# NVlabs/GLAMR

Hardware: NVIDIA H100
Metric: global_opt_frame_person_iterations_per_sec (higher is better)
Workload: dtype f32

## Files before the change

### glamr_b200/csrc/common.cuh

```cuda
#pragma once
#include <cuda_fp16.h>
#include <cuda_runtime.h>
#include <stdint.h>
#include <stdio.h>
#include <stdlib.h>

#include "../../include/glamr_b200.h"

#define GLAMR_CUDA_TRY(expr)                       \
  do {                                             \
    cudaError_t _e = (expr);                       \
    if (_e != cudaSuccess) return (int)_e;         \
  } while (0)

#define GLAMR_LAUNCH_CHECK()                       \
  do {                                             \
    cudaError_t _e = cudaGetLastError();           \
    if (_e != cudaSuccess) return (int)_e;         \
  } while (0)

#ifdef GLAMR_EXPERIMENT
#define GLAMR_DBG(x) (x)
#else
#define GLAMR_DBG(x) 0
// ... 42 lines not shown
}
__device__ __forceinline__ void mbar_fence_init() { asm volatile("fence.mbarrier_init.release.cluster;" ::: "memory"); }
__device__ __forceinline__ void mbar_expect_tx(uint64_t* bar, uint32_t bytes) {
  asm volatile("mbarrier.arrive.expect_tx.shared::cta.b64 _, [%0], %1;" ::"r"(smem_u32(bar)), "r"(bytes) : "memory");
}
__device__ __forceinline__ void mbar_expect_tx_only(uint64_t* bar, uint32_t bytes) {
  asm volatile("mbarrier.expect_tx.relaxed.cta.shared::cta.b64 [%0], %1;" ::"r"(smem_u32(bar)), "r"(bytes) : "memory");
}
__device__ __forceinline__ void mbar_arrive(uint64_t* bar) {
  asm volatile("mbarrier.arrive.shared::cta.b64 _, [%0];" ::"r"(smem_u32(bar)) : "memory");
}
__device__ __forceinline__ void mbar_wait(uint64_t* bar, uint32_t parity) {
  uint32_t ok = 0;
  const uint32_t addr = smem_u32(bar);
  while (!ok) {
    asm volatile(
        "{\n\t.reg .pred p;\n\t"
        "mbarrier.try_wait.parity.shared::cta.b64 p, [%1], %2;\n\t"
        "selp.u32 %0, 1, 0, p;\n\t}"
        : "=r"(ok)
        : "r"(addr), "r"(parity)
        : "memory");
  }
}
__device__ __forceinline__ void tma_bulk_g2s(void* smem_dst, const void* gsrc, uint32_t bytes, uint64_t* bar) {
  asm volatile("cp.async.bulk.shared::cluster.global.mbarrier::complete_tx::bytes [%0], [%1], %2, [%3];" ::"r"(smem_u32(smem_dst)),
               "l"(gsrc), "r"(bytes), "r"(smem_u32(bar))
               : "memory");
}

__device__ __forceinline__ void pdl_wait() { asm volatile("griddepcontrol.wait;" ::: "memory"); }
__device__ __forceinline__ void pdl_launch_dependents() { asm volatile("griddepcontrol.launch_dependents;" ::: "memory"); }

__device__ __forceinline__ uint64_t wgmma_desc_kmajor_noswizzle(const void* smem_ptr, int rows) {
  const uint32_t addr = smem_u32(smem_ptr);
  uint64_t d = 0;
  d |= (uint64_t)((addr >> 4) & 0x3FFF);
  d |= (uint64_t)((rows * 16) >> 4) << 16;
  d |= (uint64_t)(128 >> 4) << 32;
  return d;
}
__device__ __forceinline__ void wgmma_fence() { asm volatile("wgmma.fence.sync.aligned;" ::: "memory"); }
__device__ __forceinline__ void wgmma_commit() { asm volatile("wgmma.commit_group.sync.aligned;" ::: "memory"); }
template <int N>
__device__ __forceinline__ void wgmma_wait() { asm volatile("wgmma.wait_group.sync.aligned %0;" ::"n"(N) : "memory"); }
template <int R>
__device__ __forceinline__ void wgmma_fence_acc(float (&d)[R]) {
#pragma unroll
  for (int i = 0; i < R; ++i) asm volatile("" : "+f"(d[i])::"memory");
}
__device__ __forceinline__ void wgmma_m64n128k8_tf32(float (&d)[64], uint64_t da, uint64_t db, uint32_t accumulate) {
  asm volatile(
      "{\n\t.reg .pred p;\n\tsetp.ne.b32 p, %66, 0;\n\t"
      "wgmma.mma_async.sync.aligned.m64n128k8.f32.tf32.tf32 "
      "{%0, %1, %2, %3, %4, %5, %6, %7, %8, %9, %10, %11, %12, %13, %14, %15, %16, %17, %18, %19, %20, %21, %22, %23, %24, %25, %26, %27, %28, %29, %30, %31, %32, %33, %34, %35, %36, %37, %38, %39, %40, %41, %42, %43, %44, %45, %46, %47, %48, %49, %50, %51, %52, %53, %54, %55, %56, %57, %58, %59, %60, %61, %62, %63}, %64, %65, p, 1, 1;\n\t}\n"
      : "+f"(d[0]), "+f"(d[1]), "+f"(d[2]), "+f"(d[3]), "+f"(d[4]), "+f"(d[5]), "+f"(d[6]), "+f"(d[7]),
        "+f"(d[8]), "+f"(d[9]), "+f"(d[10]), "+f"(d[11]), "+f"(d[12]), "+f"(d[13]), "+f"(d[14]), "+f"(d[15]),
        "+f"(d[16]), "+f"(d[17]), "+f"(d[18]), "+f"(d[19]), "+f"(d[20]), "+f"(d[21]), "+f"(d[22]), "+f"(d[23]),
        "+f"(d[24]), "+f"(d[25]), "+f"(d[26]), "+f"(d[27]), "+f"(d[28]), "+f"(d[29]), "+f"(d[30]), "+f"(d[31]),
        "+f"(d[32]), "+f"(d[33]), "+f"(d[34]), "+f"(d[35]), "+f"(d[36]), "+f"(d[37]), "+f"(d[38]), "+f"(d[39]),
        "+f"(d[40]), "+f"(d[41]), "+f"(d[42]), "+f"(d[43]), "+f"(d[44]), "+f"(d[45]), "+f"(d[46]), "+f"(d[47]),
        "+f"(d[48]), "+f"(d[49]), "+f"(d[50]), "+f"(d[51]), "+f"(d[52]), "+f"(d[53]), "+f"(d[54]), "+f"(d[55]),
        "+f"(d[56]), "+f"(d[57]), "+f"(d[58]), "+f"(d[59]), "+f"(d[60]), "+f"(d[61]), "+f"(d[62]), "+f"(d[63])
      : "l"(da), "l"(db), "r"(accumulate));
}
__device__ __forceinline__ void wgmma_m64n240k8_tf32(float (&d)[120], uint64_t da, uint64_t db, uint32_t accumulate) {
// ... 53 lines not shown
        "+f"(d[96]), "+f"(d[97]), "+f"(d[98]), "+f"(d[99]), "+f"(d[100]), "+f"(d[101]), "+f"(d[102]), "+f"(d[103]),
        "+f"(d[104]), "+f"(d[105]), "+f"(d[106]), "+f"(d[107]), "+f"(d[108]), "+f"(d[109]), "+f"(d[110]), "+f"(d[111]),
        "+f"(d[112]), "+f"(d[113]), "+f"(d[114]), "+f"(d[115]), "+f"(d[116]), "+f"(d[117]), "+f"(d[118]), "+f"(d[119]),
        "+f"(d[120]), "+f"(d[121]), "+f"(d[122]), "+f"(d[123]), "+f"(d[124]), "+f"(d[125]), "+f"(d[126]), "+f"(d[127])
      : "l"(da), "l"(db), "r"(accumulate));
}


__device__ __forceinline__ void split_tf32(float x, float& hi, float& lo) {
  uint32_t h, l;
  asm("cvt.rna.tf32.f32 %0, %1;" : "=r"(h) : "f"(x));
  hi = __uint_as_float(h);
  asm("cvt.rna.tf32.f32 %0, %1;" : "=r"(l) : "f"(x - hi));
  lo = __uint_as_float(l);
}
__device__ __forceinline__ void split_f16_scaled(float x, float s, __half& hi, __half& lo) {
  const float xs = x * s;
  hi = __float2half_rn(xs);
  lo = __float2half_rn(xs - __half2float(hi));
}

__device__ __forceinline__ float warp_sum(float v) {
#pragma unroll
  for (int o = 16; o > 0; o >>= 1) v += __shfl_xor_sync(0xffffffffu, v, o);
  return v;
}
__device__ __forceinline__ double warp_sum(double v) {
#pragma unroll
  for (int o = 16; o > 0; o >>= 1) v += __shfl_xor_sync(0xffffffffu, v, o);
  return v;
}

#if defined(__CUDACC__)
constexpr int kPdlDefaultMask = 0;
inline bool pdl_enabled(int bit) {
  static int mask = -1;
  if (mask < 0) {
    const char* e = getenv("GLAMR_PDL");
    mask = e ? atoi(e) : kPdlDefaultMask;
  }
  return (mask & bit) != 0;
}
template <typename... KArgs, typename... Args>
inline cudaError_t launch_pdl(int bit, void (*kernel)(KArgs...), dim3 grid, dim3 block, size_t smem, cudaStream_t s, Args... args) {
  cudaLaunchConfig_t cfg = {};
  cfg.gridDim = grid;
  cfg.blockDim = block;
  cfg.dynamicSmemBytes = smem;
  cfg.stream = s;
  cudaLaunchAttribute attr[1];
  attr[0].id = cudaLaunchAttributeProgrammaticStreamSerialization;
  attr[0].val.programmaticStreamSerializationAllowed = 1;
  cfg.attrs = attr;
  cfg.numAttrs = pdl_enabled(bit) ? 1 : 0;
  return cudaLaunchKernelEx(&cfg, kernel, KArgs(args)...);
}
#endif

}
```

### glamr_b200/csrc/globalopt_kernels.cu

```cuda
#include <stdlib.h>
#include <algorithm>
#include <string.h>
#include <vector>

#include "globalopt_frames.cuh"
#include "smpl_model.cuh"
#include "block_scan.cuh"

namespace glamr {

constexpr int kFrameThreads = 128;

struct GroupGrid {
  int res0;
  int cam0;
  int cam30;
  int slot0;
};
struct SlotLayout {
  int res;
  int persons;
  int cam;
  int cam3;
  int n_res, n_cam, n_cam3;
// ... 21 lines not shown
}

__device__ void block_reduce_terms(const TermAcc& acc, double* out , double* smem ) {
  const int lane = threadIdx.x & 31, wid = threadIdx.x >> 5, nw = blockDim.x >> 5;
#pragma unroll
  for (int k = 0; k < GLAMR_NUM_TERMS; ++k) {
    const double s = warp_sum(acc.v[k]);
    if (lane == 0) smem[wid * GLAMR_NUM_TERMS + k] = s;
  }
  __syncthreads();
  if (threadIdx.x < GLAMR_NUM_TERMS) {
    double s = 0.0;
    for (int w = 0; w < nw; ++w) s += smem[w * GLAMR_NUM_TERMS + threadIdx.x];
    out[threadIdx.x] = s;
  }
}

__device__ bool grid_last_block(unsigned int* ticket) {
  __shared__ bool last;
  __threadfence();
  __syncthreads();
  if (threadIdx.x == 0) {
    const unsigned int old = atomicAdd(ticket, 1u);
    last = (old == gridDim.x - 1);
    if (last) *ticket = 0u;
  }
  __syncthreads();
  if (last) __threadfence();
  return last;
}

__global__ void __launch_bounds__(kScanThreads) traj_cam_forward_kernel(OptCtx c, int with_cam, SlotLayout sl) {
  __shared__ float sm[kScanThreads / 32 + 1];
  pdl_launch_dependents();
  pdl_wait();
  const int n_reduce = c.pb.n_params + num_groups(c.pb) * GLAMR_NUM_TERMS;
  for (int i = blockIdx.x * kScanThreads + threadIdx.x; i < n_reduce; i += gridDim.x * kScanThreads) c.sc.grad[i] = 0.0f;
  if ((int)blockIdx.x >= c.pb.P) {
    const int b = blockIdx.x - c.pb.P, G = num_groups(c.pb);
    const int g = G > 1 ? grid_group(sl, G, &GroupGrid::cam0, b) : 0;
    const int t = (G > 1 ? b - sl.grid[g].cam0 : b) * kScanThreads + threadIdx.x;
    if (with_cam && t < group_frames(c.pb, g)) cam_forward(c, (int)group_cam_row0(c.pb, g) + t);
    return;
  }
  const int p = blockIdx.x;
  const glamr_person_t& ps = c.pb.persons[p];
  const int len = ps.len, T = person_frames(c.pb, p);
  const size_t n0 = person_row(c.pb, p) + ps.start;
  if (c.pb.traj_source == GLAMR_TRAJ_PREDICTED) {
    for (int i = threadIdx.x; i < len; i += kScanThreads) traj_pre(c, p, i);
    __syncthreads();
    block_scan_inplace(c.sc.heading + n0, len, 1, false, sm);
    __syncthreads();
    for (int i = threadIdx.x; i < len; i += kScanThreads) traj_mid(c, p, i);
    __syncthreads();
    block_scan_inplace(c.sc.xy + 2 * n0, len, 2, false, sm);
    block_scan_inplace(c.sc.xy + 2 * n0 + 1, len, 2, false, sm);
    __syncthreads();
  }
  for (int t = threadIdx.x; t < T; t += kScanThreads) traj_post(c, p, t);
}

__global__ void __launch_bounds__(kFrameThreads) cam_forward_kernel(OptCtx c, int cam_rows) {
  pdl_launch_dependents();
  pdl_wait();
  const int gt = blockIdx.x * blockDim.x + threadIdx.x;
  if (gt < cam_rows) cam_forward(c, gt);
}

__global__ void __launch_bounds__(kFrameThreads) frame_residuals_kernel(OptCtx c, SmplDev m, SmplWorkspace wo, int n_begin, double* partial,
                                                                        SlotLayout sl) {
  __shared__ double sm[(kFrameThreads / 32) * GLAMR_NUM_TERMS];
  pdl_launch_dependents();
  pdl_wait();
  const int lane = threadIdx.x & 31, wid = threadIdx.x >> 5;
  const int G = num_groups(c.pb);
  const int g = G > 1 ? grid_group(sl, G, &GroupGrid::res0, blockIdx.x) : 0;
  const int lb = G > 1 ? blockIdx.x - sl.grid[g].res0 : blockIdx.x;
  const int T = group_frames(c.pb, g), Ng = group_persons(c.pb, g) * T, J = c.pb.J;
  const int ng = lb * (kFrameThreads / 32) + wid;
  const int n = (int)group_first_row(c.pb, g) + ng;
  GLAMR_STAMP(0);
  TermAcc acc;
  acc.clear();
  if (ng < Ng) {
    const int q = ng / T, t = ng - q * T, p = group_first_person(c.pb, g) + q;
    if (n >= c.pb.n_begin && n < c.pb.n_end) {
      const int nl = n - n_begin;
      const float* tw = c.sc.trans_world + (size_t)n * 3;
      const float sc = c.pb.scale_all ? c.pb.scale_all[n] : 1.0f;
      const float* cam = c.sc.cam + cam_row(c, p, t) * 12;
      float root[3], Rc[9], tc[3], Rs[9];
      raw_joint(m, wo, nl, m.joint_map[0], root);
      mat34_R(cam, Rc);
      tc[0] = cam[3]; tc[1] = cam[7]; tc[2] = cam[11];
      rodrigues_smplx(c.sc.orient_world + (size_t)n * 3, Rs);
      KpGrad kg;
      kg.clear();
      GLAMR_STAMP(1);
      for (int k = lane; k < J; k += 32) {
        float v[3], jw[3];
        raw_joint(m, wo, nl, m.joint_map[k], v);
        jw[0] = (v[0] - root[0]) * sc + tw[0];
        jw[1] = (v[1] - root[1]) * sc + tw[1];
        jw[2] = (v[2] - root[2]) * sc + tw[2];
        float* o = c.sc.joints_world + ((size_t)n * J + k) * 3;
        o[0] = jw[0]; o[1] = jw[1]; o[2] = jw[2];
        kp_joint_terms(c, p, t, k, jw, Rc, tc, Rs, tw, kg);
      }
      GLAMR_STAMP(2);
#pragma unroll
      for (int k = 0; k < 3; ++k) { kg.g_tc[k] = warp_sum(kg.g_tc[k]); kg.g_tw[k] = warp_sum(kg.g_tw[k]); }
#pragma unroll
      for (int k = 0; k < 9; ++k) { kg.g_Rc[k] = warp_sum(kg.g_Rc[k]); kg.g_Rs[k] = warp_sum(kg.g_Rs[k]); }
      kg.kp = warp_sum(kg.kp);
      kg.dist = warp_sum(kg.dist);
      GLAMR_STAMP(3);
      if (lane == 0) frame_rest(c, p, t, kg, acc);
      GLAMR_STAMP(10);
    } else if (lane == 0) {
      for (int k = 0; k < 3; ++k) { c.sc.g_orient[(size_t)n * 3 + k] = 0.0f; c.sc.g_trans[(size_t)n * 3 + k] = 0.0f; }
      for (int k = 0; k < 12; ++k) c.sc.g_cam[(size_t)n * 12 + k] = 0.0f;
    }
  }
  if (lane == 0)
    for (int k = 0; k < GLAMR_NUM_TERMS; ++k) sm[wid * GLAMR_NUM_TERMS + k] = acc.v[k];
  __syncthreads();
  if (threadIdx.x < GLAMR_NUM_TERMS) {
    double s = 0.0;
    for (int w = 0; w < kFrameThreads / 32; ++w) s += sm[w * GLAMR_NUM_TERMS + threadIdx.x];
    partial[((size_t)group_slot(sl, c.pb, g, 0) + lb) * GLAMR_NUM_TERMS + threadIdx.x] = s;
  }
  GLAMR_STAMP(11);
}

#ifdef GLAMR_EXPERIMENT
extern "C" int glamr_exp_frame_stamps(long long* out32) {
  GLAMR_CUDA_TRY(cudaDeviceSynchronize());
  GLAMR_CUDA_TRY(cudaMemcpyFromSymbol(out32, g_frame_stamps, sizeof(long long) * 32));
  return GLAMR_OK;
}
#endif

__global__ void __launch_bounds__(kFrameThreads) camera_backward_kernel(OptCtx c, double* partial, SlotLayout sl) {
  __shared__ double sm[(kFrameThreads / 32) * GLAMR_NUM_TERMS];
  pdl_launch_dependents();
  pdl_wait();
  const int G = num_groups(c.pb);
  const int g = G > 1 ? grid_group(sl, G, &GroupGrid::cam30, blockIdx.x) : 0;
  const int lb = G > 1 ? blockIdx.x - sl.grid[g].cam30 : blockIdx.x;
  const int t = lb * blockDim.x + threadIdx.x;
  TermAcc acc;
  acc.clear();
  if (t < group_frames(c.pb, g)) camera_backward(c, (int)group_cam_row0(c.pb, g) + t, acc);
  block_reduce_terms(acc, partial + ((size_t)group_slot(sl, c.pb, g, 3) + lb) * GLAMR_NUM_TERMS, sm);
}

__global__ void __launch_bounds__(kFrameThreads) camera_scatter_kernel(OptCtx c, int cam_rows) {
  pdl_launch_dependents();
  pdl_wait();
  const int gs = blockIdx.x * blockDim.x + threadIdx.x;
  if (gs < cam_rows) camera_scatter_to_persons(c, gs);
}

struct PeerCtx {
  int rank, world;
  size_t slot_elems;
  unsigned long long* bufs[GLAMR_MAX_PEERS];
};
// ... 35 lines not shown
    const double* pg = partial + (size_t)first * GLAMR_NUM_TERMS;
    double s = 0.0;
    for (int k = 0; k < end - first; ++k) s += pg[(size_t)k * GLAMR_NUM_TERMS + k0];
    reduce_buf[c.pb.n_params + i] = (float)s;
  }
  if (c.pb.cam_mode == GLAMR_CAM_FIXED) {
    for (int g = 0; g < G; ++g) {
      const float* gcf = c.sc.g_cam_fix + group_cam_row0(c.pb, g) * 12;
      const int T = group_frames(c.pb, g);
      double a[9];
      for (int k = 0; k < 9; ++k) a[k] = 0.0;
      for (int t = tid; t < T; t += blockDim.x)
        for (int k = 0; k < 9; ++k) a[k] += (double)gcf[(size_t)t * 12 + k];
      for (int k = 0; k < 9; ++k) {
        const double s = warp_sum(a[k]);
        if (lane == 0) sm[wid * 16 + k] = s;
      }
      __syncthreads();
      if (tid < 9) {
        double s = 0.0;
        for (int w = 0; w < (int)(blockDim.x >> 5); ++w) s += sm[w * 16 + tid];
        const int off = (tid < 6) ? group_off_cam_rot(c.pb, g) + tid : group_off_cam_trans(c.pb, g) + (tid - 6);
        reduce_buf[off] = (float)s;
      }
      __syncthreads();
    }
  }
}

__global__ void __launch_bounds__(kScanThreads, 1) traj_cam_backward_kernel(OptCtx c, int with_cam, double* partial, SlotLayout sl,
                                                                         float* reduce_buf, unsigned int* ticket, PeerCtx pc) {
  __shared__ float sm[kScanThreads / 32 + 1];
  __shared__ double smd[(kScanThreads / 32) * GLAMR_NUM_TERMS];
  pdl_launch_dependents();
  pdl_wait();
  TermAcc acc;
  acc.clear();
  size_t slot;
  if ((int)blockIdx.x >= c.pb.P) {
    const int b = blockIdx.x - c.pb.P, G = num_groups(c.pb);
    const int g = G > 1 ? grid_group(sl, G, &GroupGrid::cam0, b) : 0;
    const int lb = G > 1 ? b - sl.grid[g].cam0 : b;
    const int t = lb * kScanThreads + threadIdx.x;
    if (with_cam && t < group_frames(c.pb, g)) camera_backward(c, (int)group_cam_row0(c.pb, g) + t, acc);
    slot = (size_t)group_slot(sl, c.pb, g, 2) + lb;
  } else {
    const int p = blockIdx.x, g = person_group(c.pb, p);
    slot = (size_t)group_slot(sl, c.pb, g, 1) + (p - group_first_person(c.pb, g));
    const glamr_person_t& ps = c.pb.persons[p];
    const int len = ps.len, T = person_frames(c.pb, p);
    const size_t n0 = person_row(c.pb, p) + ps.start;
    const bool codec = c.pb.traj_source == GLAMR_TRAJ_PREDICTED;
    for (int t = threadIdx.x; t < T; t += kScanThreads) traj_back_pre(c, p, t, acc);
    __syncthreads();
    if (codec) {
      block_scan_inplace(c.sc.g_xy + 2 * n0, len, 2, true, sm);
      block_scan_inplace(c.sc.g_xy + 2 * n0 + 1, len, 2, true, sm);
      __syncthreads();
    }
    for (int i = threadIdx.x; i < len; i += kScanThreads) traj_back_mid(c, p, i, acc);
    __syncthreads();
    if (codec) {
      block_scan_inplace(c.sc.g_head + n0, len, 1, true, sm);
      __syncthreads();
    }
    for (int i = threadIdx.x; i < len; i += kScanThreads) traj_back_post(c, p, i, acc);
// ... 15 lines not shown
    float g = 0.0f;
    for (int r = 0; r < pc.world; ++r) g += peer_take(pc, epoch, r, i);
    buf[i] = g;
  }
  if (grid_last_block(ticket) && threadIdx.x == 0) reinterpret_cast<uint32_t*>(pc.bufs[pc.rank])[1] = epoch;
}

struct AdamState {
  float* m;
  float* v;
  double* beta_pow;
};

__device__ void write_losses(const OptCtx& c, int g, const float* term_sums , float* loss_terms) {
  double total = 0.0;
  for (int k = 0; k < GLAMR_NUM_TERMS; ++k) {
    float val = 0.0f;
    if (c.pb.term_enabled[k]) {
      val = term_sums[k] / term_norm(c.pb, g, k);
      if (!c.pb.term_monitor[k]) total += (double)val * (double)c.pb.term_weight[k];
    }
    loss_terms[k] = val;
  }
  loss_terms[GLAMR_NUM_TERMS] = (float)total;
}

__global__ void __launch_bounds__(32) losses_kernel(OptCtx c, const float* __restrict__ reduce_buf, float* __restrict__ loss_terms) {
  for (int g = threadIdx.x; g < num_groups(c.pb); g += blockDim.x)
    write_losses(c, g, reduce_buf + c.pb.n_params + g * GLAMR_NUM_TERMS, loss_terms + g * (GLAMR_NUM_TERMS + 1));
}

__global__ void __launch_bounds__(256) apply_kernel(OptCtx c, float* __restrict__ theta, const float* __restrict__ reduce_buf, double lr,
                                                    AdamState ad, float* loss_terms, int hist_stride, unsigned int* ticket, PeerCtx pc) {
  pdl_launch_dependents();
  pdl_wait();
  const double b1 = ad.beta_pow[0] * 0.9, b2 = ad.beta_pow[1] * 0.999, step = ad.beta_pow[2];
  const uint32_t epoch = pc.world > 1 ? reinterpret_cast<const uint32_t*>(pc.bufs[pc.rank])[1] + 1u : 0u;
  if (pc.world > 1) {
    const size_t row = peer_row(pc, epoch, pc.rank);
    const int count = c.pb.n_params + num_groups(c.pb) * GLAMR_NUM_TERMS;
    for (int i = blockIdx.x * blockDim.x + threadIdx.x; i < count; i += gridDim.x * blockDim.x) {
      const unsigned long long w = ((unsigned long long)epoch << 32) | (unsigned long long)__float_as_uint(reduce_buf[i]);
      for (int r = 0; r < pc.world; ++r) st_peer_u64(pc.bufs[r] + row + i, w);
    }
  }
  auto grad_at = [&](int i) -> float {
    if (pc.world <= 1) return reduce_buf[i];
    float g = 0.0f;
    for (int r = 0; r < pc.world; ++r) g += peer_take(pc, epoch, r, i);
    return g;
  };
  for (int g = threadIdx.x; blockIdx.x == 0 && g < num_groups(c.pb) && loss_terms; g += blockDim.x) {
    float sums[GLAMR_NUM_TERMS];
    for (int k = 0; k < GLAMR_NUM_TERMS; ++k) sums[k] = grad_at(c.pb.n_params + g * GLAMR_NUM_TERMS + k);
    write_losses(c, g, sums, loss_terms + (hist_stride > 0 ? (size_t)step * hist_stride : 0) + g * (GLAMR_NUM_TERMS + 1));
  }
  const float bc2s = (float)sqrt(1.0 - b2);
  const float step_size = (float)(lr / (1.0 - b1));
  for (int i = blockIdx.x * blockDim.x + threadIdx.x; i < c.pb.n_params; i += gridDim.x * blockDim.x) {
    if (!c.pb.active[i]) continue;
    const float g = grad_at(i);
    float m = ad.m[i], v = ad.v[i];
    m = m + 0.1f * (g - m);
    v = v * 0.999f + 0.001f * g * g;
    const float denom = sqrtf(v) / bc2s + 1e-8f;
    theta[i] = theta[i] - step_size * (m / denom);
// ... 633 lines not shown
```

### glamr_b200/csrc/smpl_kernels.cu

```cuda
#include <math.h>
#include <algorithm>
#include <cmath>
#include <stdlib.h>
#include <string.h>

#include <vector>

#include "glamr_math.cuh"
#include "smpl_model.cuh"

namespace glamr {

__global__ void __launch_bounds__(128) pose_prep_kernel(SmplDev m, int n, const float* __restrict__ orient,
                                                        const float* __restrict__ body_pose,
                                                        const float* __restrict__ betas, int use_betas, SmplWorkspace w) {
  pdl_launch_dependents();
  pdl_wait();
  const int f = (blockIdx.x * blockDim.x + threadIdx.x) >> 5;
  if (f >= n) return;
  pose_prep_frame(m, f, orient ? orient + (size_t)f * 3 : nullptr, body_pose + (size_t)f * 69, use_betas ? betas + (size_t)f * kNB : nullptr, w,
                  threadIdx.x & 31);
}

constexpr int kFramesPerCta = 32;
constexpr int kFramesPerWarp = 8;
constexpr int kVertsPerThread = 4;
constexpr int kLbsThreads = 128;
constexpr int kMaxStages = 4;
constexpr int kChunkFloats = kChunkK * kTileCols;
constexpr uint32_t kChunkBytes = kChunkFloats * sizeof(float);
constexpr int kPfChunkFloats = kChunkK * kFramesPerCta;
constexpr uint32_t kPfChunkBytes = kPfChunkFloats * sizeof(float);
constexpr int kATileFloats = kFramesPerCta * kNJ * 12;
constexpr int kVpFloats = kVTile * 3 * kFramesPerCta;
__host__ __device__ constexpr int stage_region_floats(int stages) { return (stages * (kChunkFloats + kPfChunkFloats) > kVpFloats) ? stages * (kChunkFloats + kPfChunkFloats) : kVpFloats; }
constexpr size_t lbs_smem_bytes(int stages) { return (size_t)(stage_region_floats(stages) + kATileFloats + kFramesPerCta * kNB) * sizeof(float) + (2 * kMaxStages + 1) * sizeof(uint64_t); }

template <int KREG, int kStages>
__global__ void __launch_bounds__(kLbsThreads, 2)
lbs_kernel(SmplDev m, int n_begin, int n_end, const float* __restrict__ betas, SmplWorkspace w, float* __restrict__ vertices, int dbg) {
  constexpr int kStageRegionFloats = stage_region_floats(kStages);
  extern __shared__ __align__(128) unsigned char smem_raw[];
  float* PDs = reinterpret_cast<float*>(smem_raw);
  float* pfs = PDs + kStages * kChunkFloats;
  float* As = PDs + kStageRegionFloats;
  float* bs = As + kATileFloats;
  uint64_t* full = reinterpret_cast<uint64_t*>(bs + kFramesPerCta * kNB);
  uint64_t* empty = full + kStages;
  uint64_t* abar = empty + kStages;

  const int tid = threadIdx.x;
  const int lane = tid & 31;
  const int wf = (tid >> 5) * kFramesPerWarp;
  const int vtile = blockIdx.x;
// ... 182 lines not shown
        const int ci = m.compact_of_vertex[gv];
        const int pos = ((((fr >> 2) ^ ((vi >> 2) & 7)) << 2) | (fr & 3));
        const float x = VP[(vi * 3 + 0) * 32 + pos], y = VP[(vi * 3 + 1) * 32 + pos], z = VP[(vi * 3 + 2) * 32 + pos];
        float T[12];
#pragma unroll
        for (int k = 0; k < 12; ++k) T[k] = 0.0f;
        for (int s = 0; s < m.K; ++s) {
          const int jj = m.skin_j[(size_t)gv * m.K + s];
          const float wt = m.skin_w[(size_t)gv * m.K + s];
          const float* a = As + (jj * 32 + fr) * 12;
#pragma unroll
          for (int k = 0; k < 12; ++k) T[k] = fmaf(wt, a[k], T[k]);
        }
        const float ox = fmaf(T[0], x, fmaf(T[1], y, fmaf(T[2], z, T[3])));
        const float oy = fmaf(T[4], x, fmaf(T[5], y, fmaf(T[6], z, T[7])));
        const float oz = fmaf(T[8], x, fmaf(T[9], y, fmaf(T[10], z, T[11])));
        if (n_ok) {
          if (vertices) {
            float* o = vertices + ((size_t)n * kV + gv) * 3;
            o[0] = ox; o[1] = oy; o[2] = oz;
          }
          if (ci >= 0) {
            float* o = w.vcompact + ((size_t)n * m.S + ci) * 3;
            o[0] = ox; o[1] = oy; o[2] = oz;
          }
        }
      }
    }
  }
}


__global__ void __launch_bounds__(128) blend_features_kernel(int n, const float* __restrict__ body_pose, const float* __restrict__ betas, SmplWorkspace w) {
  const int f = (blockIdx.x * blockDim.x + threadIdx.x) >> 5, lane = threadIdx.x & 31;
  if (f >= n) return;
  float R[9];
  if (lane >= 1 && lane < kNJ) {
    const float* bp = body_pose + (size_t)f * 69 + (lane - 1) * 3;
    const float rv[3] = {bp[0], bp[1], bp[2]};
    rodrigues_smplx(rv, R);
  }
  put_blend_features(w, f, lane, R, betas ? betas + (size_t)f * kNB : nullptr);
}

constexpr int kTcStages = 8;
constexpr int kTcThreads = 288;
constexpr uint32_t kTcABytes = kTcAStageHalves * sizeof(__half);
constexpr uint32_t kTcBBytes = kTcBStageHalves * sizeof(__half);
constexpr size_t kTcRingBytes = (size_t)kTcStages * (kTcABytes + kTcBBytes) + 128;
constexpr size_t kTcSmemBytes = kTcRingBytes + 2 * (size_t)kTcOutCols * kTcOutPitch * sizeof(float);

#ifdef GLAMR_EXPERIMENT
constexpr int kBlendPhaseCtas = 1024;
constexpr int kBlendPhases = 5;
__device__ unsigned long long g_blend_phases[kBlendPhaseCtas][2][kBlendPhases];
#define BLEND_CLOCK_INIT() long long bl_ph[kBlendPhases] = {}; long long bl_t = clock64()
#define BLEND_CLOCK(k) do { const long long bl_now = clock64(); bl_ph[k] += bl_now - bl_t; bl_t = bl_now; } while (0)
#define BLEND_CLOCK_TILE() (++bl_ph[kBlendPhases - 1])
#define BLEND_CLOCK_STORE() do { if ((warp & 3) == 0 && lane == 0 && blockIdx.x < kBlendPhaseCtas)                                     \
      for (int k = 0; k < kBlendPhases; ++k) atomicAdd(&g_blend_phases[blockIdx.x][g][k], (unsigned long long)bl_ph[k]); } while (0)
extern "C" int glamr_exp_blend_phases(long long* out) {
  void* p = nullptr;
  GLAMR_CUDA_TRY(cudaDeviceSynchronize());
  GLAMR_CUDA_TRY(cudaMemcpyFromSymbol(out, g_blend_phases, sizeof(g_blend_phases)));
  GLAMR_CUDA_TRY(cudaGetSymbolAddress(&p, g_blend_phases));
  GLAMR_CUDA_TRY(cudaMemset(p, 0, sizeof(g_blend_phases)));
  return GLAMR_OK;
}
#else
#define BLEND_CLOCK_INIT() do { } while (0)
#define BLEND_CLOCK(k) do { } while (0)
#define BLEND_CLOCK_TILE() do { } while (0)
#define BLEND_CLOCK_STORE() do { } while (0)
#endif

__device__ __forceinline__ void warpgroup_sync(int g) {
  if (g == 0) asm volatile("bar.sync 1, 128;" ::: "memory");
  else asm volatile("bar.sync 2, 128;" ::: "memory");
}

__global__ void __launch_bounds__(kTcThreads, 1) lbs_blend_tc_kernel(SmplDev m, SmplWorkspace w, int mtile0, int mtiles, int half_last, int ntn) {
  extern __shared__ __align__(128) unsigned char tc_raw[];
  __half* As = reinterpret_cast<__half*>(tc_raw);
  __half* Bs = As + kTcStages * kTcAStageHalves;
  uint64_t* full = reinterpret_cast<uint64_t*>(Bs + kTcStages * kTcBStageHalves);
  uint64_t* empty = full + kTcStages;
  const int tid = threadIdx.x, warp = tid >> 5, lane = tid & 31;
  const int ntiles = ntn * mtiles;
  pdl_launch_dependents();
  if (tid == 0) {
#pragma unroll
    for (int s = 0; s < kTcStages; ++s) { mbar_init(&full[s], 1); mbar_init(&empty[s], 8); }
    mbar_fence_init();
  }
  __syncthreads();

  if (warp == 8) {
    if (lane == 0) {
      {
        const __half* gB = m.tcB + (size_t)(blockIdx.x / mtiles) * kTcChunks * kTcBStageHalves;
        for (int c = 0; c < kTcStages; ++c) {
          mbar_expect_tx_only(&full[c], kTcBBytes);
          tma_bulk_g2s(Bs + c * kTcBStageHalves, gB + (size_t)c * kTcBStageHalves, kTcBBytes, &full[c]);
        }
      }
      pdl_wait();
      int q = 0;
      for (int t = blockIdx.x; t < ntiles; t += gridDim.x) {
        const __half* gA = w.tcA + (size_t)(mtile0 + t % mtiles) * kTcChunks * kTcAStageHalves;
        const __half* gB = m.tcB + (size_t)(t / mtiles) * kTcChunks * kTcBStageHalves;
        for (int c = 0; c < kTcChunks; ++c, ++q) {
          const int s = q % kTcStages;
          if (q >= kTcStages) {
            mbar_wait(&empty[s], ((q / kTcStages) - 1) & 1);
            mbar_expect_tx(&full[s], kTcABytes + kTcBBytes);
            tma_bulk_g2s(Bs + s * kTcBStageHalves, gB + (size_t)c * kTcBStageHalves, kTcBBytes, &full[s]);
          } else {
            mbar_expect_tx(&full[s], kTcABytes);
          }
          tma_bulk_g2s(As + s * kTcAStageHalves, gA + (size_t)c * kTcAStageHalves, kTcABytes, &full[s]);
        }
// ... 171 lines not shown
          const int jj = m.skin_j[(size_t)gv * m.K + sidx];
          const float wt = m.skin_w[(size_t)gv * m.K + sidx];
          const float* a = As + (jj * 32 + fr) * 12;
#pragma unroll
          for (int k = 0; k < 12; ++k) T[k] = fmaf(wt, a[k], T[k]);
        }
      }
      const float ox = fmaf(T[0], x[u], fmaf(T[1], y[u], fmaf(T[2], z[u], T[3])));
      const float oy = fmaf(T[4], x[u], fmaf(T[5], y[u], fmaf(T[6], z[u], T[7])));
      const float oz = fmaf(T[8], x[u], fmaf(T[9], y[u], fmaf(T[10], z[u], T[11])));
      if (n_ok) {
        if (vertices) {
          float* o = vertices + ((size_t)n * kV + gv) * 3;
          o[0] = ox; o[1] = oy; o[2] = oz;
        }
        if (ci >= 0) {
          float* o = w.vcompact + ((size_t)n * m.S + ci) * 3;
          o[0] = ox; o[1] = oy; o[2] = oz;
        }
      }
    }
  }
}


constexpr uint32_t kSkWBytes = kSkWImageFloats * sizeof(float);
constexpr uint32_t kSkBBytes = kSkBImageFloats * sizeof(float);
constexpr uint32_t kSkVBytes = kSkVpTileFloats * sizeof(float);
constexpr size_t kSkinTcSmemBytes = (size_t)kSkWBytes + 2 * kSkBBytes + 2 * kSkVBytes + 128;

constexpr int kSkinTcThreads = 288;

#ifdef GLAMR_EXPERIMENT
constexpr int kSkinPhaseCtas = 1024;
constexpr int kSkinPhases = 6;
__device__ long long g_skin_phases[kSkinPhaseCtas][2][kSkinPhases];
#define SKIN_CLOCK_INIT() long long sk_ph[kSkinPhases] = {}; long long sk_t = clock64()
#define SKIN_CLOCK(k) do { const long long sk_now = clock64(); sk_ph[k] += sk_now - sk_t; sk_t = sk_now; } while (0)
#define SKIN_CLOCK_STORE(items) do { sk_ph[kSkinPhases - 1] = (items);                                                              \
    if ((warp & 3) == 0 && lane == 0 && blockIdx.x < kSkinPhaseCtas)                                                               \
      for (int k = 0; k < kSkinPhases; ++k) g_skin_phases[blockIdx.x][g][k] = sk_ph[k]; } while (0)
extern "C" int glamr_exp_skin_phases(long long* out) {
  void* p = nullptr;
  GLAMR_CUDA_TRY(cudaDeviceSynchronize());
  GLAMR_CUDA_TRY(cudaMemcpyFromSymbol(out, g_skin_phases, sizeof(g_skin_phases)));
  GLAMR_CUDA_TRY(cudaGetSymbolAddress(&p, g_skin_phases));
  GLAMR_CUDA_TRY(cudaMemset(p, 0, sizeof(g_skin_phases)));
  return GLAMR_OK;
}
#else
#define SKIN_CLOCK_INIT() do { } while (0)
#define SKIN_CLOCK(k) do { } while (0)
#define SKIN_CLOCK_STORE(items) do { } while (0)
#endif

__global__ void __launch_bounds__(kSkinTcThreads, 1) lbs_skin_tc_kernel(SmplDev m, int n, SmplWorkspace w, float* __restrict__ vertices,
                                                                        int vt0, int vt1) {
  extern __shared__ __align__(128) unsigned char sk_raw[];
  float* Ws = reinterpret_cast<float*>(sk_raw);
  float* Bs = Ws + kSkWImageFloats;
  float* Vs = Bs + 2 * kSkBImageFloats;
  uint64_t* full_w = reinterpret_cast<uint64_t*>(Vs + 2 * kSkVpTileFloats);
  uint64_t* full_b = full_w + 1;
  uint64_t* b_empty = full_w + 3;
  uint64_t* full_v = full_w + 5;
  uint64_t* v_empty = full_w + 7;
  const int tid = threadIdx.x, warp = tid >> 5, lane = tid & 31;
  const int nft = (n + kSkF - 1) / kSkF;
  const int items = (vt1 - vt0) * nft;
  const int i0 = (int)((long long)blockIdx.x * items / gridDim.x), i1 = (int)((long long)(blockIdx.x + 1) * items / gridDim.x);
  pdl_launch_dependents();
  if (tid == 0) {
    mbar_init(full_w, 1);
    for (int b = 0; b < 2; ++b) {
      mbar_init(&full_b[b], 1);
      mbar_init(&b_empty[b], 8);
      mbar_init(&full_v[b], 1);
      mbar_init(&v_empty[b], 8);
    }
    mbar_fence_init();
  }
  __syncthreads();

  if (warp == 8) {
    if (lane == 0) {
      mbar_expect_tx(full_w, kSkWBytes);
      tma_bulk_g2s(Ws, m.skW + (size_t)(vt0 + i0 / nft) * kSkWImageFloats, kSkWBytes, full_w);
      pdl_wait();
      const float* const vpb = vp_buffer(w);
      for (int i = i0, it = 0; i < i1; ++i, ++it) {
        const int vtile = vt0 + i / nft, ftile = i - (vtile - vt0) * nft, vb = it & 1;
        const bool new_w = it > 0 && ftile == 0;
        if (it >= 2) mbar_wait(&b_empty[vb], ((it - 2) >> 1) & 1);
        if (new_w) mbar_wait(&b_empty[vb ^ 1], ((it - 1) >> 1) & 1);
        mbar_expect_tx(&full_b[vb], kSkBBytes + (new_w ? kSkWBytes : 0u));
        tma_bulk_g2s(Bs + vb * kSkBImageFloats, w.skB + (size_t)ftile * kSkBImageFloats, kSkBBytes, &full_b[vb]);
        if (new_w) tma_bulk_g2s(Ws, m.skW + (size_t)vtile * kSkWImageFloats, kSkWBytes, &full_b[vb]);
        if (it >= 2) mbar_wait(&v_empty[vb], ((it - 2) >> 1) & 1);
        mbar_expect_tx(&full_v[vb], kSkVBytes);
        tma_bulk_g2s(Vs + vb * kSkVpTileFloats, vpb + ((size_t)ftile * w.vp_cols + (size_t)vtile * kTileCols) * kSkF, kSkVBytes, &full_v[vb]);
      }
    }
    return;
// ... 560 lines not shown
```

### glamr_b200/csrc/smpl_model.cuh

```cuda
#pragma once
#include "common.cuh"
#include "glamr_math.cuh"

namespace glamr {

struct SmplDev {
  const float* pd_tiles;
  const __half* tcB;
  float tcB_unscale;
  int tc_ntiles;
  const float* skW;
  int sk_tiles;
  const float* v_template;
  const float* shapedirs;
  const float* j_template;
  const float* j_shapedirs;
  const float* skin_w;
  const uint8_t* skin_j;
  int K;
  const int32_t* compact_of_vertex;
  int S;
  const int32_t* reg_ptr;
  const int32_t* reg_ci;
  const float* reg_w;
// ... 82 lines not shown
  };
  if (lane >= 1 && lane < kNJ) {
#pragma unroll
    for (int k = 0; k < 9; ++k) put((lane - 1) * 9 + k, R[k] - ((k % 4 == 0) ? 1.0f : 0.0f));
  } else if (lane == 0) {
#pragma unroll
    for (int l = 0; l < kNB; ++l) put(kPF + l, beta ? beta[l] : 0.0f);
    put(kPF + kNB, 1.0f);
#pragma unroll
    for (int k = kTcFeat; k < kTcK; ++k) put(k, 0.0f);
    w.tcUnscale[f] = ldexpf(1.0f, -e);
  }
}

__device__ __forceinline__ void raw_joint(const SmplDev& m, const SmplWorkspace& w, int f, int idx, float* o) {
  if (idx < kNJ) {
    const float* p = w.jposed + ((size_t)f * kNJ + idx) * 3;
    o[0] = p[0]; o[1] = p[1]; o[2] = p[2];
  } else if (idx < kNJ + m.n_picks) {
    const float* p = w.vcompact + ((size_t)f * m.S + m.pick_ci[idx - kNJ]) * 3;
    o[0] = p[0]; o[1] = p[1]; o[2] = p[2];
  } else {
    const int r = idx - kNJ - m.n_picks;
    float a0 = 0.f, a1 = 0.f, a2 = 0.f;
    for (int e = m.reg_ptr[r]; e < m.reg_ptr[r + 1]; ++e) {
      const float* p = w.vcompact + ((size_t)f * m.S + m.reg_ci[e]) * 3;
      const float wt = m.reg_w[e];
      a0 = fmaf(wt, p[0], a0); a1 = fmaf(wt, p[1], a1); a2 = fmaf(wt, p[2], a2);
    }
    o[0] = a0; o[1] = a1; o[2] = a2;
  }
}

__device__ __forceinline__ void pose_prep_frame(const SmplDev& m, int f, const float* __restrict__ orient3, const float* __restrict__ bp,
                                                const float* __restrict__ beta, const SmplWorkspace& w, int lane) {
  const int j = lane < kNJ ? lane : kNJ - 1;
  float r[3];
  if (j == 0) {
    r[0] = orient3 ? orient3[0] : 0.0f;
    r[1] = orient3 ? orient3[1] : 0.0f;
    r[2] = orient3 ? orient3[2] : 0.0f;
  } else {
    const float* q = bp + (j - 1) * 3;
    r[0] = q[0]; r[1] = q[1]; r[2] = q[2];
  }
  float R[9];
  rodrigues_smplx(r, R);
  float J[3];
#pragma unroll
  for (int c = 0; c < 3; ++c) {
    float v = m.j_template[j * 3 + c];
    if (beta) {
      const float* js = m.j_shapedirs + (j * 3 + c) * kNB;
#pragma unroll
      for (int l = 0; l < kNB; ++l) v = fmaf(js[l], beta[l], v);
    }
    J[c] = v;
  }
  if (lane >= 1 && lane < kNJ) {
    float* pf = w.pf + (((size_t)(f >> 5) * kNChunks + (lane - 1)) * kChunkK) * 32 + (f & 31);
#pragma unroll
    for (int k = 0; k < 9; ++k) pf[k * 32] = R[k] - ((k % 4 == 0) ? 1.0f : 0.0f);
  }
  if (w.tcA) put_blend_features(w, f, lane, R, beta);

  float GR[9], Gt[3];
#pragma unroll
  for (int k = 0; k < 9; ++k) GR[k] = R[k];
#pragma unroll
  for (int k = 0; k < 3; ++k) Gt[k] = J[k];
  const int par = m.parents[j] < 0 ? 0 : m.parents[j];
  const int lev = m.level[j];
  for (int l = 1; l < m.n_levels; ++l) {
    float pR[9], pt[3], pJ[3];
#pragma unroll
    for (int k = 0; k < 9; ++k) pR[k] = __shfl_sync(0xffffffffu, GR[k], par);
#pragma unroll
    for (int k = 0; k < 3; ++k) pt[k] = __shfl_sync(0xffffffffu, Gt[k], par);
#pragma unroll
    for (int k = 0; k < 3; ++k) pJ[k] = __shfl_sync(0xffffffffu, J[k], par);
    if (lev == l) {
      float nR[9], rel[3], nt[3];
      mat3_mul(pR, R, nR);
      rel[0] = J[0] - pJ[0]; rel[1] = J[1] - pJ[1]; rel[2] = J[2] - pJ[2];
      mat3_vec(pR, rel, nt);
#pragma unroll
      for (int k = 0; k < 9; ++k) GR[k] = nR[k];
#pragma unroll
// ... 48 lines not shown
```

Before: 2.866 million.

## Enable PDL by default and prefetch pose-prep inputs before the grid dependency wait

Programmatic dependent launch is now on by default for two launch groups (mask bits 2 and 4). This lets successive kernels overlap their launch and prologue with the tail of the previous kernel. The pose-prep kernel now loads body pose, joint template, joint shapedirs and betas into registers before griddepcontrol.wait, so those global loads overlap the predecessor. It also adds span-timing instrumentation that only compiles under GLAMR_EXPERIMENT. The risk is that body_pose or betas may be written by the preceding optimizer step, so reading them before the wait could return stale parameters. The larger register struct may also lower occupancy.

```diff
diff --git a/glamr_b200/csrc/common.cuh b/glamr_b200/csrc/common.cuh
--- a/glamr_b200/csrc/common.cuh
+++ b/glamr_b200/csrc/common.cuh
@@ -98,6 +98,50 @@
 __device__ __forceinline__ void pdl_wait() { asm volatile("griddepcontrol.wait;" ::: "memory"); }
 __device__ __forceinline__ void pdl_launch_dependents() { asm volatile("griddepcontrol.launch_dependents;" ::: "memory"); }
 
+enum SpanId { kSpanTrajFwd, kSpanPosePrep, kSpanSkinSupport, kSpanSkinMesh, kSpanResiduals, kSpanTrajBwd, kSpanApply, kSpanBlendFeat,
+              kSpanBlendGemm, kNumSpans };
+#ifdef GLAMR_EXPERIMENT
+static __device__ unsigned long long g_spans[kNumSpans][4];
+__device__ __forceinline__ unsigned long long globaltimer_ns() {
+  unsigned long long t;
+  asm volatile("mov.u64 %0, %%globaltimer;" : "=l"(t));
+  return t;
+}
+__device__ __forceinline__ bool first_active_lane() { return (int)(threadIdx.x & 31) == __ffs(__activemask()) - 1; }
+struct SpanGuard {
+  int k;
+  __device__ explicit SpanGuard(int id) : k(id) {
+    if (threadIdx.x == 0) atomicMin(&g_spans[k][0], globaltimer_ns());
+  }
+  __device__ void waited() const {
+    if (first_active_lane()) {
+      const unsigned long long t = globaltimer_ns();
+      atomicMin(&g_spans[k][1], t);
+      atomicMax(&g_spans[k][2], t);
+    }
+  }
+  __device__ ~SpanGuard() {
+    if (first_active_lane()) atomicMax(&g_spans[k][3], globaltimer_ns());
+  }
+};
+#define GLAMR_SPAN(k) const glamr::SpanGuard glamr_span_guard_(k)
+#define GLAMR_SPAN_WAITED() glamr_span_guard_.waited()
+#define GLAMR_SPANS_ENTRY(name)                                                                                        \
+  extern "C" int name(unsigned long long* out, int reset) {                                                            \
+    GLAMR_CUDA_TRY(cudaDeviceSynchronize());                                                                           \
+    if (out) GLAMR_CUDA_TRY(cudaMemcpyFromSymbol(out, glamr::g_spans, sizeof(glamr::g_spans)));                        \
+    if (reset) {                                                                                                       \
+      unsigned long long init[glamr::kNumSpans][4];                                                                    \
+      for (int k = 0; k < glamr::kNumSpans; ++k) { init[k][0] = init[k][1] = ~0ull; init[k][2] = init[k][3] = 0ull; } \
+      GLAMR_CUDA_TRY(cudaMemcpyToSymbol(glamr::g_spans, init, sizeof(init)));                                          \
+    }                                                                                                                  \
+    return GLAMR_OK;                                                                                                   \
+  }
+#else
+#define GLAMR_SPAN(k) do { } while (0)
+#define GLAMR_SPAN_WAITED() do { } while (0)
+#endif
+
 __device__ __forceinline__ uint64_t wgmma_desc_kmajor_noswizzle(const void* smem_ptr, int rows) {
   const uint32_t addr = smem_u32(smem_ptr);
   uint64_t d = 0;
@@ -217,7 +261,7 @@
 }
 
 #if defined(__CUDACC__)
-constexpr int kPdlDefaultMask = 0;
+constexpr int kPdlDefaultMask = 2 | 4;
 inline bool pdl_enabled(int bit) {
   static int mask = -1;
   if (mask < 0) {
diff --git a/glamr_b200/csrc/globalopt_kernels.cu b/glamr_b200/csrc/globalopt_kernels.cu
--- a/glamr_b200/csrc/globalopt_kernels.cu
+++ b/glamr_b200/csrc/globalopt_kernels.cu
@@ -77,8 +77,10 @@
 
 __global__ void __launch_bounds__(kScanThreads) traj_cam_forward_kernel(OptCtx c, int with_cam, SlotLayout sl) {
   __shared__ float sm[kScanThreads / 32 + 1];
+  GLAMR_SPAN(kSpanTrajFwd);
   pdl_launch_dependents();
   pdl_wait();
+  GLAMR_SPAN_WAITED();
   const int n_reduce = c.pb.n_params + num_groups(c.pb) * GLAMR_NUM_TERMS;
   for (int i = blockIdx.x * kScanThreads + threadIdx.x; i < n_reduce; i += gridDim.x * kScanThreads) c.sc.grad[i] = 0.0f;
   if ((int)blockIdx.x >= c.pb.P) {
@@ -116,6 +118,7 @@
 __global__ void __launch_bounds__(kFrameThreads) frame_residuals_kernel(OptCtx c, SmplDev m, SmplWorkspace wo, int n_begin, double* partial,
                                                                         SlotLayout sl) {
   __shared__ double sm[(kFrameThreads / 32) * GLAMR_NUM_TERMS];
+  GLAMR_SPAN(kSpanResiduals);
   pdl_launch_dependents();
   pdl_wait();
   const int lane = threadIdx.x & 31, wid = threadIdx.x >> 5;
@@ -180,6 +183,7 @@
 }
 
 #ifdef GLAMR_EXPERIMENT
+GLAMR_SPANS_ENTRY(glamr_exp_spans_opt)
 extern "C" int glamr_exp_frame_stamps(long long* out32) {
   GLAMR_CUDA_TRY(cudaDeviceSynchronize());
   GLAMR_CUDA_TRY(cudaMemcpyFromSymbol(out32, g_frame_stamps, sizeof(long long) * 32));
@@ -281,6 +285,7 @@
                                                                          float* reduce_buf, unsigned int* ticket, PeerCtx pc) {
   __shared__ float sm[kScanThreads / 32 + 1];
   __shared__ double smd[(kScanThreads / 32) * GLAMR_NUM_TERMS];
+  GLAMR_SPAN(kSpanTrajBwd);
   pdl_launch_dependents();
   pdl_wait();
   TermAcc acc;
@@ -362,6 +367,7 @@
 
 __global__ void __launch_bounds__(256) apply_kernel(OptCtx c, float* __restrict__ theta, const float* __restrict__ reduce_buf, double lr,
                                                     AdamState ad, float* loss_terms, int hist_stride, unsigned int* ticket, PeerCtx pc) {
+  GLAMR_SPAN(kSpanApply);
   pdl_launch_dependents();
   pdl_wait();
   const double b1 = ad.beta_pow[0] * 0.9, b2 = ad.beta_pow[1] * 0.999, step = ad.beta_pow[2];
diff --git a/glamr_b200/csrc/smpl_kernels.cu b/glamr_b200/csrc/smpl_kernels.cu
--- a/glamr_b200/csrc/smpl_kernels.cu
+++ b/glamr_b200/csrc/smpl_kernels.cu
@@ -14,12 +14,16 @@
 __global__ void __launch_bounds__(128) pose_prep_kernel(SmplDev m, int n, const float* __restrict__ orient,
                                                         const float* __restrict__ body_pose,
                                                         const float* __restrict__ betas, int use_betas, SmplWorkspace w) {
+  GLAMR_SPAN(kSpanPosePrep);
   pdl_launch_dependents();
+  const int f = (blockIdx.x * blockDim.x + threadIdx.x) >> 5, lane = threadIdx.x & 31;
+  if (f >= n) return;
+  const float* beta = use_betas ? betas + (size_t)f * kNB : nullptr;
+  PosePrepIn in;
+  pose_prep_load(m, body_pose + (size_t)f * 69, beta, lane, in);
   pdl_wait();
-  const int f = (blockIdx.x * blockDim.x + threadIdx.x) >> 5;
-  if (f >= n) return;
-  pose_prep_frame(m, f, orient ? orient + (size_t)f * 3 : nullptr, body_pose + (size_t)f * 69, use_betas ? betas + (size_t)f * kNB : nullptr, w,
-                  threadIdx.x & 31);
+  GLAMR_SPAN_WAITED();
+  pose_prep_frame(m, f, orient ? orient + (size_t)f * 3 : nullptr, in, beta, w, lane);
 }
 
 constexpr int kFramesPerCta = 32;
@@ -268,6 +272,7 @@
 
 
 __global__ void __launch_bounds__(128) blend_features_kernel(int n, const float* __restrict__ body_pose, const float* __restrict__ betas, SmplWorkspace w) {
+  GLAMR_SPAN(kSpanBlendFeat);
   const int f = (blockIdx.x * blockDim.x + threadIdx.x) >> 5, lane = threadIdx.x & 31;
   if (f >= n) return;
   float R[9];
@@ -323,6 +328,7 @@
   uint64_t* empty = full + kTcStages;
   const int tid = threadIdx.x, warp = tid >> 5, lane = tid & 31;
   const int ntiles = ntn * mtiles;
+  GLAMR_SPAN(kSpanBlendGemm);
   pdl_launch_dependents();
   if (tid == 0) {
 #pragma unroll
@@ -560,6 +566,10 @@
 constexpr int kSkinTcThreads = 288;
 
 #ifdef GLAMR_EXPERIMENT
+GLAMR_SPANS_ENTRY(glamr_exp_spans_smpl)
+#endif
+
+#ifdef GLAMR_EXPERIMENT
 constexpr int kSkinPhaseCtas = 1024;
 constexpr int kSkinPhases = 6;
 __device__ long long g_skin_phases[kSkinPhaseCtas][2][kSkinPhases];
@@ -597,6 +607,7 @@
   const int nft = (n + kSkF - 1) / kSkF;
   const int items = (vt1 - vt0) * nft;
   const int i0 = (int)((long long)blockIdx.x * items / gridDim.x), i1 = (int)((long long)(blockIdx.x + 1) * items / gridDim.x);
+  GLAMR_SPAN(vt0 >= kNVTiles ? kSpanSkinSupport : kSpanSkinMesh);
   pdl_launch_dependents();
   if (tid == 0) {
     mbar_init(full_w, 1);
diff --git a/glamr_b200/csrc/smpl_model.cuh b/glamr_b200/csrc/smpl_model.cuh
--- a/glamr_b200/csrc/smpl_model.cuh
+++ b/glamr_b200/csrc/smpl_model.cuh
@@ -138,7 +138,31 @@
   }
 }
 
-__device__ __forceinline__ void pose_prep_frame(const SmplDev& m, int f, const float* __restrict__ orient3, const float* __restrict__ bp,
+struct PosePrepIn {
+  float q[3];
+  float jt[3];
+  float js[3][kNB];
+  float beta[kNB];
+};
+__device__ __forceinline__ void pose_prep_load(const SmplDev& m, const float* __restrict__ bp, const float* __restrict__ beta, int lane,
+                                               PosePrepIn& in) {
+  const int j = lane < kNJ ? lane : kNJ - 1;
+#pragma unroll
+  for (int k = 0; k < 3; ++k) in.q[k] = j == 0 ? 0.0f : bp[(j - 1) * 3 + k];
+#pragma unroll
+  for (int c = 0; c < 3; ++c) {
+    in.jt[c] = m.j_template[j * 3 + c];
+    if (beta) {
+#pragma unroll
+      for (int l = 0; l < kNB; ++l) in.js[c][l] = m.j_shapedirs[(j * 3 + c) * kNB + l];
+    }
+  }
+  if (beta) {
+#pragma unroll
+    for (int l = 0; l < kNB; ++l) in.beta[l] = beta[l];
+  }
+}
+__device__ __forceinline__ void pose_prep_frame(const SmplDev& m, int f, const float* __restrict__ orient3, const PosePrepIn& in,
                                                 const float* __restrict__ beta, const SmplWorkspace& w, int lane) {
   const int j = lane < kNJ ? lane : kNJ - 1;
   float r[3];
@@ -147,19 +171,17 @@
     r[1] = orient3 ? orient3[1] : 0.0f;
     r[2] = orient3 ? orient3[2] : 0.0f;
   } else {
-    const float* q = bp + (j - 1) * 3;
-    r[0] = q[0]; r[1] = q[1]; r[2] = q[2];
+    r[0] = in.q[0]; r[1] = in.q[1]; r[2] = in.q[2];
   }
   float R[9];
   rodrigues_smplx(r, R);
   float J[3];
 #pragma unroll
   for (int c = 0; c < 3; ++c) {
-    float v = m.j_template[j * 3 + c];
+    float v = in.jt[c];
     if (beta) {
-      const float* js = m.j_shapedirs + (j * 3 + c) * kNB;
-#pragma unroll
-      for (int l = 0; l < kNB; ++l) v = fmaf(js[l], beta[l], v);
+#pragma unroll
+      for (int l = 0; l < kNB; ++l) v = fmaf(in.js[c][l], in.beta[l], v);
     }
     J[c] = v;
   }
```

Measured after the change: 2.871 million, median of 6. About the same (+0.2%).
